# MPI-SWS/RedQueen

Hardware: AMD Instinct MI355X
Metric: redqueen_replicas_per_sec (higher is better)
Workload: dtype f64; 1 GPU; C3 syn1k: 1000 followers, 50 sources (25 Poisson2 rate 1 + 25 Hawkes l0=1 a=1 b=10), degree 5, T=100, q=1e6, s=1, RedQueen, randomized worlds; replicas_per_gpu=10000, global_batch=10000, parallelism=replica-sharded dp1, replicas_per_chunk=10000

## Files before the change

redqueen_amd/csrc/rq_api.cpp:

```cpp
#include <hip/hip_runtime.h>

#include <algorithm>
#include <cstring>
#include <memory>
#include <mutex>
#include <new>
#include <vector>

#include "../../include/rq.h"
#include "rq_internal.h"

using rqh::align_up;
using rqh::CtrlTables;
using rqh::GraphTopo;
using rqh::Knobs;
using rqh::Plan;

namespace {

template <class T>
struct DevBuf {
    T* p = nullptr;
    size_t n = 0;
    ~DevBuf() { if (p) (void)hipFree(p); }
// ... 562 lines not shown
    if (!g || !ids) return RQ_EINVAL;
    std::copy(g->fol_ids.begin(), g->fol_ids.end(), ids);
    return RQ_OK;
}

int rq_workspace_size(rq_graph_t g, const rq_batch_desc* b, size_t* bytes)
{
    if (!bytes) return RQ_EINVAL;
    Plan p;
    const int rc = plan_call(g, b, rqh::read_knobs(), 0.0, &p);
    if (rc) return rc;
    *bytes = p.total;
    return RQ_OK;
}

int rq_plan_info(rq_graph_t g, const rq_batch_desc* b, int64_t* info)
{
    return rq_plan_info_n(g, b, info, 8);
}

int rq_plan_info_n(rq_graph_t g, const rq_batch_desc* b, int64_t* out, int n)
{
    if (!out || n < 0) return RQ_EINVAL;
    int64_t info[10];
    Plan p;
    const int rc = plan_call(g, b, rqh::read_knobs(), 0.0, &p);
    if (rc) return rc;
    rqh::plan_info(p, b->ctrl_kind, info);
    info[9] = p.blk ? 1 : 0;
    std::copy(info, info + std::min(n, 10), out);
    return RQ_OK;
}

int rq_event_capacity(rq_graph_t g, const rq_batch_desc* b, int64_t* cap)
{
    if (!cap) return RQ_EINVAL;
    Plan p;
    const int rc = plan_call(g, b, rqh::read_knobs(), 0.0, &p);
    if (rc) return rc;
    *cap = p.cap_rows;
    return RQ_OK;
}

int rq_run_batch(rq_graph_t g, const rq_batch_desc* b, const rq_outputs* out, void* workspace,
                 size_t workspace_bytes, void* hip_stream)
{
    const Knobs kn = rqh::read_knobs();
    Plan p;
    int rc = plan_call(g, b, kn, (double)workspace_bytes, &p);
    if (rc) return rc;
    if (!out || !out->metrics || !out->counts || !out->status || !workspace) return RQ_EINVAL;
    if (workspace_bytes < p.total) return RQ_EINVAL;
    if ((b->flags & RQ_RUN_EVENT_LOG) && (!out->ev_t || !out->ev_src || out->ev_cap < 1))
// ... 4 lines not shown
    if ((rc = stage_tables(g, p, b, rqh::ctrl_tables(*g, b), ws, pst[0]))) return rc;
    if (hipMemsetAsync(out->status, 0, sizeof(int32_t) * p.R, pst[0]) != hipSuccess) return RQ_EHIP;
    Join join{pst, t_pipes.of(pst[0])};
    if ((rc = fork_streams(p.nbuf, &join))) return rc;

    int64_t ci = 0;
    for (int64_t c0 = 0; c0 < p.R; c0 += p.chunk, ++ci) {
        hipStream_t s = pst[ci % p.nbuf];
        const Chunk ch{c0, std::min(p.chunk, p.R - c0), ws,
                       ws + p.off_set0 + (size_t)(ci % p.nbuf) * p.set_stride};
        const GenArgs ga = gen_args(g, p, b, out, ch, kn);
        if (!p.fw || p.fwm) {
            TimedLaunch tl(K_GEN, s);
            if (rq_launch_gen(ga, s) != hipSuccess) return RQ_EHIP;
        }
        if (p.mrg && (rc = launch_merge(p, merge_args(g, p, out, ch, ga, kn), ch, s))) return rc;
        const SweepArgs sa = sweep_args(g, p, b, out, ch, ga, kn);
        if (p.order && rq_launch_order(sa.mrg_len, ch.C, (int*)(ch.wsb + p.off_ord), s) != hipSuccess)
            return RQ_EHIP;
        if (hipMemsetAsync(ch.wsb + p.off_wq, 0, 2 * sizeof(int), s) != hipSuccess) return RQ_EHIP;
        {
            TimedLaunch tl(K_SWEEP, s);
            const SweepInst inst = rqh::sweep_inst(p, b->ctrl_kind);
            const hipError_t e = inst.fused ? rq_launch_sweep_fw(sa, inst, s) : rq_launch_sweep(sa, inst, s);
            if (e != hipSuccess) return RQ_EHIP;
        }
        if (p.scan) continue;
        const ScanArgs sc = scan_args(g, p, out, ch, sa);
        TimedLaunch tl(K_SCAN, s);
        if (rq_launch_scan(sc, p.nK, s) != hipSuccess) return RQ_EHIP;
    }
    return join.done();
}

int rq_timing(int enable)
{
    for (int k = 0; k < K_N; ++k) {
        for (auto& e : g_ev[k]) {
            (void)hipEventDestroy(e.first);
            (void)hipEventDestroy(e.second);
        }
        g_ev[k].clear();
    }
    g_timing = enable != 0;
    return RQ_OK;
}

// ... 762 lines not shown
```

redqueen_amd/csrc/rq_host.h:

```cpp
#pragma once
#include <stddef.h>
#include <stdint.h>

#include <vector>

#include "../../include/rq.h"

#define RQ_MAX_STREAMS 2048
#define RQ_NPSUM1_LDS 516
#ifndef RQ_MRG_LB
#define RQ_MRG_LB 1024
#endif
#define RQ_MG_B 512
#define RQ_MAX_STREAMS_MRG (RQ_MG_B * RQ_MG_B)

struct SweepInst {
    bool fused;
    int nK;
    bool col16;
    bool log;
    bool gs;
    bool bits;
    bool bl;
    bool mrg;
    int spl;
    int W;
    bool gt;
    bool pw;
    bool pair;
    bool scan;
    bool blk;
};
#define RQ_BLK_CB(nw) ((((nw) + 7) >> 3) << 1)
#define RQ_BLK_MSTRIDE(nw) (4 * RQ_BLK_CB(nw) + 4)
#define RQ_BLK_MIN_NW 13
#define RQ_FWS_NL 66
#define RQ_FWS_LDS_BYTES(nK) ((size_t)8 * (((nK) + 2 + 3) * RQ_FWS_NL + 4))

#ifndef RQ_FOLLOWERS_TILE_SINKS
#define RQ_FOLLOWERS_TILE_SINKS 2048
#endif
static_assert(RQ_FOLLOWERS_TILE_SINKS >= 1 &&
                  (long long)RQ_FOLLOWERS_TILE_SINKS * (12 + 8 * (RQ_MAX_K + 2) + 8) <= 160 * 1024,
              "a tile of every nK / rows variant must fit one workgroup's LDS");

int rq_sweep_blocks_per_cu(const SweepInst& i, int wpb, size_t lds);
int rq_fw_blocks_per_cu(const SweepInst& i, int wpb, size_t lds);
int rq_cu_count();

namespace rqh {

inline size_t align_up(size_t x, size_t a) { return (x + a - 1) / a * a; }

inline int followers_tiles(int n_sinks) { return (n_sinks + RQ_FOLLOWERS_TILE_SINKS - 1) / RQ_FOLLOWERS_TILE_SINKS; }
inline size_t followers_tiled_ws_bytes(int n_sinks, int64_t n_rep)
{
    return align_up((size_t)4 * (size_t)n_rep * (size_t)followers_tiles(n_sinks), 256);
}

template <class T>
struct Knob {
    bool set = false;
    T v{};
};
struct Knobs {
    Knob<double> ws_budget_gb;
    double cap_squeeze = 1.0;
    Knob<int> mg_grp;
    bool mrg = true;
    Knob<int> g_collds;
    int g_w = 0;
    bool skip = true;
    bool fwm = true;
    bool ctrl_draws = true;
    bool sweep_scan = true;
    bool gen_split = true;
    bool phasec_blk = true;
    int fw_w = 0;
    int pipe = 2;
    Knob<int64_t> pipe_chunk;
    bool order = false;

    int sweep_dbg = 0;
    double fw_tile = 58.0;
    Knob<int> fw_hmin, fw_thr, fw_hfill;
    int fw_static = 0;
    bool clk_merge = false;

    Knob<int> rp_chunk;
    bool rp_small = true;
    bool clk_replay = false;

    int lm_of_slots = 4096;
};
Knobs read_knobs();

struct GraphTopo {
    int n_str = 0, ctrl_idx = -1, n_sinks = 0, n_fol = 0;
// ... 31 lines not shown
    std::vector<int> cap;
    std::vector<int64_t> st_off;
    std::vector<int> rd_k;
    bool log = false, bits = false;
    bool bl = false;
    size_t g_fb = 0, g_etab = 0, g_inv = 0, g_skip = 0;
    bool g_inv_sh = false;
    bool gs = false;
    int64_t gs_slots = 0, gs_stride = 0;
    bool fw = false;
    int fw_h = 8, mstride = 1;
    bool mrg = false;
    bool lmrg = false;
    bool gt = false;
    size_t off_mt = 0, off_mj = 0, off_mjh = 0, off_mlen = 0;
    int64_t mrg_stride = 0;
    int n_grp = 1;
    int grp_sz = RQ_MG_B;
    int64_t sub_stride = 0;
    size_t off_sub_t = 0, off_sub_j = 0, off_sub_len = 0;
    bool fwm = false;
    bool pair = false;
    bool scan = false;
    bool blk = false;
    int gwpb = 4, gwin = 16, gcol_lds = 1, gcol16 = 0;
    size_t g_col = 0, g_ptr = 0, g_odf = 0, g_cbf = 0, g_wave = 0, g_wave_stride = 0, g_rank_off = 0,
           g_win_off = 0, g_x_off = 0, g_total = 0, g_stage_off = 0;
    size_t tables_bytes = 0;
    int wpc = 0;
    int nbuf = 1;
    bool order = false;
    size_t off_set0 = 0, set_stride = 0, off_ord = 0;
    size_t off_pwc = 0, off_pwmax = 0;
    size_t off_invc = 0, off_streams = 0, off_slen = 0, off_rt = 0, off_rs = 0, off_rv = 0,
           off_rc = 0, off_sall = 0, off_wq = 0, off_stoff = 0, off_cap = 0, off_rdk = 0, off_repidx = 0, off_gs = 0,
           total = 0;
};

int make_plan(const GraphTopo& g, const rq_batch_desc* b, const Knobs& kn, double budget, Plan* p);
SweepInst sweep_inst(const Plan& p, int ctrl_kind);
void plan_info(const Plan& p, int ctrl_kind, int64_t info[9]);

struct CtrlTables {
    std::vector<double> invc;
    std::vector<double> pwc, pwmax;
};
// ... 35 lines not shown
```

redqueen_amd/csrc/rq_internal.h:

```cpp
#pragma once
#include <hip/hip_runtime.h>
#include <stdint.h>

#include <map>
#include <mutex>
#include <tuple>

#include "../../include/rq.h"
#include "rq_host.h"
#include "rq_log_walk.h"

__host__ __device__ __forceinline__ int64_t rq_global_replica(int64_t s, int64_t n_rep, int64_t rep_lo,
                                                               int64_t rep_cnt)
{
    return rep_cnt == n_rep ? s : (s / rep_cnt) * n_rep + rep_lo + s % rep_cnt;
}

struct GenArgs {
    int64_t n_chunk, chunk0, rep0;
    int64_t n_rep, rep_lo, rep_cnt;
    const int64_t* rep_idx;
    int n_str, ctrl_idx, ctrl_stream_kind, randomize;
    int64_t seed_mod;
    const uint32_t* ctrl_seed;
// ... 135 lines not shown
    int64_t n_chunk, chunk0;
    const int64_t* nrows;
    int64_t nrows_stride;
    const int* sall;
    int64_t row_stride;
    const double* rows_t;
    const double* rows_sum;
    const uint32_t* rows_valid;
    const uint32_t* rows_cnt;
    double end;
    double* metrics;
    int* wq;
};

using SweepKernel = void (*)(SweepArgs);

hipError_t rq_launch_gen(const GenArgs& a, hipStream_t s);
hipError_t rq_launch_sweep(const SweepArgs& a, const SweepInst& i, hipStream_t s);
hipError_t rq_launch_scan(const ScanArgs& a, int nK, hipStream_t s);
hipError_t rq_launch_merge(const MergeArgs& a, hipStream_t s);
hipError_t rq_launch_merge_groups(const MergeArgs& a, hipStream_t s);
hipError_t rq_launch_merge_sub(const MergeArgs& a, hipStream_t s);
hipError_t rq_launch_order(const int* len, int64_t n, int* order, hipStream_t s);
hipError_t rq_launch_sweep_fw(const SweepArgs& a, const SweepInst& i, hipStream_t s);

template <class K>
int rq_occupancy(K kernel, int threads, size_t lds)
{
    static std::mutex mu;
    static std::map<std::tuple<const void*, int, size_t>, int> cache;
    const auto key = std::make_tuple(reinterpret_cast<const void*>(kernel), threads, lds);
    std::lock_guard<std::mutex> lock(mu);
    const auto it = cache.find(key);
    if (it != cache.end()) return it->second;
    int nb = 0;
    if (hipOccupancyMaxActiveBlocksPerMultiprocessor(&nb, kernel, threads, lds) != hipSuccess) nb = 0;
    cache.emplace(key, nb);
    return nb;
}

struct RpInfo {
    int64_t n_piv;
    int64_t n_own, n_world;
    int32_t S;
    int32_t flags;
};
#define RP_FALLBACK 1
// ... 277 lines not shown
```

redqueen_amd/csrc/rq_plan.cpp:

```cpp
#include <algorithm>
#include <cmath>
#include <cstdlib>

#include "rq_host.h"
#include "rq_tables.h"

namespace rqh {

Knobs read_knobs()
{
    Knobs k;
    if (const char* e = getenv("RQ_WS_BUDGET_GB")) k.ws_budget_gb = {true, atof(e)};
    if (const char* e = getenv("RQ_CAP_SQUEEZE")) k.cap_squeeze = std::max(0.01, std::min(1.0, atof(e)));
    if (const char* e = getenv("RQ_MG_GRP")) k.mg_grp = {true, atoi(e)};
    if (const char* e = getenv("RQ_MRG")) k.mrg = atoi(e) != 0;
    if (const char* e = getenv("RQ_G_COLLDS")) k.g_collds = {true, atoi(e)};
    if (const char* e = getenv("RQ_G_W")) k.g_w = atoi(e);
    if (const char* e = getenv("RQ_SKIP")) k.skip = atoi(e) != 0;
    if (const char* e = getenv("RQ_FWM")) k.fwm = atoi(e) != 0;
    if (const char* e = getenv("RQ_CTRL_DRAWS")) k.ctrl_draws = atoi(e) != 0;
    if (const char* e = getenv("RQ_SWEEP_SCAN")) k.sweep_scan = atoi(e) != 0;
    if (const char* e = getenv("RQ_GEN_SPLIT")) k.gen_split = atoi(e) != 0;
    if (const char* e = getenv("RQ_PHASEC_BLK")) k.phasec_blk = atoi(e) != 0;
    if (const char* e = getenv("RQ_FW_W")) k.fw_w = atoi(e);
    if (const char* e = getenv("RQ_PIPE")) k.pipe = std::max(1, std::min(3, atoi(e)));
    if (const char* e = getenv("RQ_PIPE_CHUNK")) k.pipe_chunk = {true, std::max<int64_t>(64, atoll(e))};
    if (const char* e = getenv("RQ_ORDER")) k.order = atoi(e) != 0;
    if (const char* e = getenv("RQ_SWEEP_DBG")) k.sweep_dbg = atoi(e);
    if (const char* e = getenv("RQ_FW_TILE")) k.fw_tile = atof(e);
    if (const char* e = getenv("RQ_FW_HMIN")) k.fw_hmin = {true, atoi(e)};
    if (const char* e = getenv("RQ_FW_THR")) k.fw_thr = {true, atoi(e)};
    if (const char* e = getenv("RQ_FW_HFILL")) k.fw_hfill = {true, atoi(e)};
    static const int fw_static = getenv("RQ_FW_STATIC") ? atoi(getenv("RQ_FW_STATIC")) : 0;
    k.fw_static = fw_static;
    k.clk_merge = getenv("RQ_CLK_MERGE") != nullptr;
    if (const char* e = getenv("RQ_RP_CHUNK")) k.rp_chunk = {true, atoi(e)};
    if (const char* e = getenv("RQ_RP_SMALL")) k.rp_small = atoi(e) != 0;
    k.clk_replay = getenv("RQ_CLK_REPLAY") != nullptr;
    if (const char* e = getenv("RQ_LM_OF_SLOTS")) k.lm_of_slots = std::max(1, std::min(4096, atoi(e)));
    return k;
}

namespace {

// ... 42 lines not shown
        break;
    }
    return m;
}

SweepInst sweep_inst(const Plan& p, int ctrl_kind, bool fused, int W, bool col16, bool gs, bool gt)
{
    SweepInst i{};
    i.fused = fused;
    i.nK = p.nK;
    i.col16 = col16;
    i.log = p.log;
    i.gs = gs;
    i.bits = p.bits;
    i.bl = p.bl;
    i.mrg = fused ? p.fwm : p.mrg;
    i.spl = p.spl;
    i.W = W;
    i.gt = gt;
    i.pw = ctrl_kind == RQ_SRC_OPTPW;
    i.pair = fused && i.mrg && p.pair;
    i.scan = fused && i.mrg && p.scan;
    i.blk = fused && i.mrg && p.blk;
    return i;
}
int sweep_blocks_per_cu(const SweepInst& i, int wpb, size_t lds)
{
    return i.fused ? rq_fw_blocks_per_cu(i, wpb, lds) : rq_sweep_blocks_per_cu(i, wpb, lds);
}

void plan_layout(const GraphTopo* g, const rq_batch_desc* b, Plan* p);

int plan_args(const GraphTopo* g, const rq_batch_desc* b, Plan* p)
{
    if (!b) return RQ_EINVAL;
    if (b->nK < 1 || b->nK > RQ_MAX_K || !b->Ks) return RQ_EINVAL;
    if (b->n_grid < 1 || b->n_rep < 1) return RQ_EINVAL;
    const int ck = b->ctrl_kind;
    if (ck != RQ_SRC_OPT && ck != RQ_SRC_OPTPW && ck != RQ_SRC_POISSON2 && ck != RQ_SRC_PWCONST &&
        ck != RQ_SRC_REALDATA && ck != RQ_SRC_NONE)
        return RQ_EINVAL;
    if (ck == RQ_SRC_OPT && (!b->q || (g->n_fol > 0 && !b->s))) return RQ_EINVAL;
    if (ck == RQ_SRC_OPTPW &&
        (!b->q || b->n_seg < 1 || b->n_seg > 4096 || !(b->period > 0.0) || (g->n_fol > 0 && !b->s_pw)))
        return RQ_EINVAL;
    if (ck == RQ_SRC_POISSON2 && !b->ctrl_rate) return RQ_EINVAL;
// ... 218 lines not shown
            if (p->scan) stride = std::max(stride, align_up(RQ_FWS_LDS_BYTES(p->nK), 16));
            for (int wpb : {16, 12, 10, 8, 6, 5, 4, 3, 2, 1}) {
                const size_t tot = sh + wpb * stride;
                if (tot > kLdsMax) continue;
                int blocks = sweep_blocks_per_cu(sweep_inst(*p, b->ctrl_kind, true, W, c16, false, false), wpb, tot);
                if (blocks <= 0) blocks = (int)std::min<size_t>(kLdsMax / tot, 16 / wpb);
                const int waves = blocks * wpb;
                const int score = waves * 4 + (W == 16 ? 2 : W == 32 ? 1 : 0);
                if (score > best) {
                    best = score;
                    p->wpc = waves;
                    p->gwin = W; p->fw_h = H; p->gwpb = wpb; p->gcol_lds = c16; p->gcol16 = c16;
                    p->g_col = o_col; p->g_ptr = o_ptr; p->g_odf = o_odf; p->g_cbf = o_cbf;
                    p->g_wave = sh; p->g_wave_stride = stride; p->g_rank_off = r_off;
                    p->g_win_off = w_off; p->g_stage_off = s_off; p->g_x_off = 0; p->g_total = tot;
                    p->g_etab = o_etab;
                }
            }
        }
        if (best < 0) p->fw = false;
    }
    if (!p->fw) p->fwm = false;
    if (!p->fwm) p->pair = p->scan = p->blk = false;
    if (p->blk) p->mstride = mstride;
    if (p->fw) p->mrg = p->fwm;
}

}

SweepInst sweep_inst(const Plan& p, int ctrl_kind)
{
    return sweep_inst(p, ctrl_kind, p.fw, p.gwin, p.gcol16, p.gs, p.gt);
}

void plan_info(const Plan& p, int ctrl_kind, int64_t info[9])
{
    info[0] = (p.log ? (p.gs ? 4 : 1) : (p.bits ? 2 : (p.bl ? 3 : 0))) + (p.fwm ? 20 : p.fw ? 10 : 0);
    info[1] = p.mrg ? 0 : p.spl;
    info[2] = p.gwin;
    info[3] = p.gwpb;
    info[4] = sweep_blocks_per_cu(sweep_inst(p, ctrl_kind), p.gwpb, p.g_total);
    info[5] = p.gcol_lds;
    info[6] = (int64_t)p.g_total;
    info[7] = p.chunk;
    info[8] = p.scan ? 1 : 0;
}
// ... 133 lines not shown
```

redqueen_amd/csrc/rq_scan_rows.h:

```cpp
#pragma once
#include <hip/hip_runtime.h>
#include <stdint.h>

#include "rq_device.h"

#pragma clang fp contract(off)

namespace rq {

template <int NK, int TU, int NL = 128>
__device__ __forceinline__ void scan_rows(int64_t n, double S, double end, const double* Rt, const double* Rs,
                                          const uint32_t* Rv, const uint32_t* Rc, double* lds,
                                          double res[NK + 2])
{
    constexpr int NV = NK + 2;
    struct Row {
        double t, s;
        uint32_t v, c[NK];
    };
    auto ld = [&](uint32_t kk) {
        Row r;
        r.t = Rt[kk];
        r.s = Rs[kk];
        r.v = Rv[kk];
#pragma unroll
        for (int q = 0; q < NK; ++q) r.c[q] = Rc[kk * NK + q];
        return r;
    };
    auto tld = [&](uint32_t kk) { return Rt[kk]; };
    auto vf = [&](const Row& r, double t1, double* v) {
        const double dt = t1 - r.t;
        const double m = r.s / (double)r.v;
#pragma unroll
        for (int q = 0; q < NK; ++q) v[q] = ((double)r.c[q] / S) * dt;
        v[NK] = m * dt;
        v[NK + 1] = (m * m) * dt;
    };
    wave_npsum_rows<NV, true, Row, TU, NL>(n, end, ld, tld, vf, lds, res);
}

}
```

redqueen_amd/csrc/rq_sweep_core.h:

```cpp
#pragma once
#include "rq_device.h"
#include "rq_internal.h"

namespace rq {
static_assert(npsum_lds_doubles<1>() == RQ_NPSUM1_LDS, "wave_npsum<1> scratch size (rq_api.cpp plans it)");

template <int NK>
struct Agg {
    int64_t sumR, sumF;
    int nvalid;
    int cnt[NK];
    int km1[NK];
    __device__ __forceinline__ void init(const int* Ks)
    {
        sumR = 0;
        sumF = 0;
        nvalid = 0;
#pragma unroll
        for (int q = 0; q < NK; ++q) {
            cnt[q] = 0;
            km1[q] = Ks[q] - 1;
        }
    }
    template <class RT, class CF>
// ... 260 lines not shown
            nvalid += popc(__ballot(nv));
            nfrac += popc(__ballot(fup)) - popc(__ballot(fdn));
#pragma unroll
            for (int q = 0; q < NK; ++q) cnt[q] += popc(__ballot(up[q])) - popc(__ballot(dn[q]));
#pragma unroll
            for (int o = 32; o > 0; o >>= 1) dsum += __shfl_xor(dsum, o, 64);
            sumI += dsum;
        }
    }
    __device__ __forceinline__ double row_sum(int n_sinks, double* lds)
    {
        if (nfrac == 0) return (double)sumI;
        double out[1];
        wave_npsum<1>((int64_t)n_sinks,
                      [&](int64_t kk, double* v) {
                          const int c = (int)kk;
                          v[0] = gtag[c] >= 0 ? (double)gsum[c] / (double)gcnt[c] : 0.0;
                      },
                      lds, out);
        return out[0];
    }
};

template <int NK>
struct RowStage {
    double r_t, r_sum;
    int r_valid;
    int r_cnt[NK];
    int64_t nrow, s0, cap;
    double last_t;
    double* Rt0;
    double* Rs0;
    uint32_t* Rv0;
    uint32_t* Rc0;
    int64_t rb;
    uint32_t p_o, p_w;
    double p_ot, p_os, p_wt, p_ws;
    int p_ov, p_wv;
    int p_oc[NK], p_wc[NK];
    __device__ __forceinline__ void init(double* t, double* s, uint32_t* v, uint32_t* c, int64_t rb_,
                                         int64_t cap_)
    {
        p_o = p_w = ~0u;
        r_t = 0.0;
        r_sum = 0.0;
        r_valid = 0;
#pragma unroll
// ... 34 lines not shown
#pragma unroll
            for (int q = 0; q < NK; ++q) r_cnt[q] = cnt[q];
        }
        ++nrow;
        last_t = t;
        if (slot == 63) {
            store(s0 + lane);
            s0 = nrow;
        }
        return true;
    }
    __device__ __forceinline__ void store(int64_t rr) { write(rr, r_t, r_sum, r_valid, r_cnt); }
    __device__ __forceinline__ void flush_pend()
    {
        if (p_o != ~0u) write(p_o, p_ot, p_os, p_ov, p_oc);
        if (p_w != ~0u) write(p_w, p_wt, p_ws, p_wv, p_wc);
        p_o = p_w = ~0u;
    }
    __device__ __forceinline__ void flush(int lane)
    {
        const int rem = (int)(nrow - s0);
        if (lane < rem) store(s0 + lane);
        s0 = nrow;
    }
};

__device__ __forceinline__ double optpw_sample(double tt, const double* row, double smax, int S,
                                               double T, uint64_t e, uint32_t oseed)
{
    if (!(smax > 0.0)) return RQ_INF;
    const double inv = 1.0 / smax;
    const double ph = fmod(tt, T);
    double ns = 0.0;
    for (uint32_t it = 1; it < (1u << 20); ++it) {
        uint32_t w4[4] = {(uint32_t)e, (uint32_t)(e >> 32), it, 0u};
        philox4x32_10(w4, oseed, kind_salt(RQ_SRC_OPTPW, true));
        ns = ns + rq_std_exponential(rq_uniform53(w4[0], w4[1])) * inv;
        int idx = (int)(((double)S * fmod(ns + ph, T)) / T);
        idx = idx < S ? idx : S - 1;
        if (rq_uniform53(w4[2], w4[3]) * smax < row[idx]) return tt + ns;
    }
    return RQ_INF;
}

template <bool PW, bool XIN = false>
__device__ __forceinline__ void controller_tile(int n, bool act, double tt, int tj, const double* invc,
// ... 44 lines not shown
}

__device__ __forceinline__ bool truncate_tile(int64_t M, int64_t n_events, int& n, bool& act, double& tt,
                                              int& tj, uint64_t& ownm, double ot, double& opt_next)
{
    if (M < 0) return false;
    const int lane = lane_id();
    const int64_t pp = n_events + lane + mbcnt64(ownm);
    const int64_t pw = pp + (int64_t)((ownm >> lane) & 1ull);
    const int nk = __popcll(__ballot(act && pw < M));
    if (nk >= n) return false;
    const bool lone = ((ownm >> nk) & 1ull) != 0ull && bcast_i64(pp, nk) < M;
    opt_next = lone ? bcast_d(ot, nk) : RQ_INF;
    ownm &= nk > 0 ? (~0ull >> (64 - nk)) : 0ull;
    n = nk;
    act = lane < nk;
    if (!act) {
        tt = RQ_INF;
        tj = 0;
    }
    return true;
}

template <int NK, bool DEFER = false>
__device__ __forceinline__ bool place_rows(RowStage<NK>& rs, uint64_t ma, bool has_o, bool has_w, double ot,
                                           double tt, int64_t osum, int oval, const int* ocnt,
                                           int64_t wsum, int wval, const int* wcnt, int& status)
{
    const int lane = lane_id();
    const uint64_t mo = __ballot(has_o), mw = __ballot(has_w);
    const uint64_t above = lane < 63 ? ma >> (lane + 1) : 0ull;
    const bool nxt = above != 0;
    const double ft = has_o ? ot : tt;
    const double nft = __shfl(ft, nxt ? lane + __ffsll((unsigned long long)above) : lane, 64);
    const bool keep_o = has_o && !(has_w ? ot == tt : (nxt && ot == nft));
    const bool keep_w = has_w && !(nxt && tt == nft);
    const bool tie0 = rs.nrow > 0 && bcast_d(ft, __ffsll((unsigned long long)ma) - 1) == rs.last_t;
    const uint64_t ko = __ballot(keep_o), kw = __ballot(keep_w);
    if (tie0 || ko != mo || kw != mw) status |= RQ_ST_TIE;
    const int64_t r0 = rs.nrow - (tie0 ? 1 : 0);
    const int64_t po = r0 + mbcnt64(ko) + mbcnt64(kw);
    const int64_t pw = po + (keep_o ? 1 : 0);
    if constexpr (DEFER) {
        rs.p_o = keep_o && po < rs.cap ? (uint32_t)po : ~0u;
        rs.p_w = keep_w && pw < rs.cap ? (uint32_t)pw : ~0u;
        rs.p_ot = ot;
        rs.p_os = (double)osum;
        rs.p_ov = oval;
        rs.p_wt = tt;
        rs.p_ws = (double)wsum;
        rs.p_wv = wval;
#pragma unroll
        for (int q = 0; q < NK; ++q) {
            rs.p_oc[q] = ocnt[q];
            rs.p_wc[q] = wcnt[q];
        }
    } else {
        if (keep_o && po < rs.cap) rs.write(po, ot, (double)osum, oval, ocnt);
        if (keep_w && pw < rs.cap) rs.write(pw, tt, (double)wsum, wval, wcnt);
    }
    rs.last_t = bcast_d(has_w ? tt : ot, 63 - __builtin_clzll(ma));
    rs.nrow = r0 + __popcll(ko) + __popcll(kw);
    rs.s0 = rs.nrow;
    if (rs.nrow > rs.cap) {
        rs.nrow = rs.cap;
        rs.s0 = rs.cap;
// ... 52 lines not shown
```

redqueen_amd/csrc/rq_sweep_fw.hip:

```cpp
#include <hip/hip_runtime.h>
#include <stdint.h>

#include "rq_device.h"
#include "rq_internal.h"
#include "rq_sweep_core.h"
#include "rq_gen.h"
#include "rq_scan_rows.h"
#include <type_traits>
#include <cstdlib>

#pragma clang fp contract(off)

using namespace rq;

constexpr int fws_tu(int nk) { return nk == 1 ? 4 : 2; }
template <int NK>
__device__ __forceinline__ void fw_scan_rows(int64_t n, double S, double end, const double* Rt, const double* Rs,
                                             const uint32_t* Rv, const uint32_t* Rc, double* lds, double* out)
{
    constexpr int NV = NK + 2;
    static_assert(RQ_FWS_LDS_BYTES(NK) == 8 * (size_t)npsum_lds_doubles<NV, RQ_FWS_NL>(), "the planner's size");
    const int lane = lane_id();
    if (n == 0) {
        if (lane < NV) out[lane] = __builtin_nan("");
        return;
    }
    __asm__ volatile("s_waitcnt vmcnt(0)" ::: "memory");
    __builtin_amdgcn_fence(__ATOMIC_RELEASE, "workgroup");
    __builtin_amdgcn_fence(__ATOMIC_ACQUIRE, "workgroup");
    double res[NV];
    scan_rows<NK, fws_tu(NK), RQ_FWS_NL>(n, S, end, Rt, Rs, Rv, Rc, lds, res);
    if (lane == 0) {
#pragma unroll
        for (int s = 0; s < NV; ++s) out[s] = res[s];
    }
}
template <int NK, class COL, int W, int H, bool BITS, bool PW, bool MRG, bool PAIR = false, bool SCAN = false,
          bool BLK = false>
__device__ __forceinline__ void sweep_fw_body(SweepArgs a)
{
    static_assert((W & (W - 1)) == 0 && H <= W, "ring");
    static_assert(!SCAN || MRG, "the sweep's own scan: merged instances only");
    static_assert(!BLK || (MRG && BITS), "event-blocked phase C: the merged sink-bit instances only");
    extern __shared__ double lds_g[];
    char* base = reinterpret_cast<char*>(lds_g);
    const int lane = lane_id();
    const int w = threadIdx.x >> 6;
    int* cptr = reinterpret_cast<int*>(base + a.lds_ptr);
    int* odf = reinterpret_cast<int*>(base + a.lds_odf);
    int* cbf = reinterpret_cast<int*>(base + a.lds_cbf);
    constexpr bool col_lds = sizeof(COL) == 2;
    COL* col_l = reinterpret_cast<COL*>(base + a.lds_col);
    const int* col_g = a.csr_col;
    if (col_lds && !BITS)
        for (int e = threadIdx.x; e < a.n_csr; e += blockDim.x) col_l[e] = (COL)a.csr_col[e];
    uint32_t* msk = reinterpret_cast<uint32_t*>(base + a.lds_mask);
    const int ms = a.mstride;
    if (BITS)
        for (int e = threadIdx.x; e < (a.n_str + 1) * ms; e += blockDim.x) {
            const int jj = e / ms, ww = e - jj * ms;
            msk[e] = (jj < a.n_str && ww < a.nw) ? a.masks[jj * a.nw + ww] : 0u;
        }
    uint64_t* etab = reinterpret_cast<uint64_t*>(base + a.lds_etab);
    for (int e = threadIdx.x; e < RQ_EXP_TAB_N; e += blockDim.x) etab[e] = rq_exp_tab_c[e];
    for (int j = threadIdx.x; j <= a.n_str; j += blockDim.x) cptr[j] = a.csr_ptr[j];
    for (int j = threadIdx.x; j < a.n_str; j += blockDim.x) {
// ... 13 lines not shown
    const int64_t rl = a.order ? (int64_t)a.order[qi] : qi;
    const int64_t o = a.chunk0 + rl;
    const int64_t i = rq_replica_of(a.gen, o);
    const int g = (int)(i / a.n_rep);
    for (int j = lane; j < a.n_str; j += 64) invc[j] = a.inv_c[(int64_t)g * a.n_str + j];
    if (!BITS)
        for (int c = lane; c < a.n_sinks; c += 64) rank[c] = -1;
    wave_lds_sync();

#ifdef RQ_PHASE_CLOCK
    unsigned long long ck[8] = {0, 0, 0, 0, 0, 0, 0, 0};
    unsigned long long tk = __builtin_amdgcn_s_memtime();
#define RQ_CLK(q)                                                   \
    do {                                                            \
        const unsigned long long t2 = __builtin_amdgcn_s_memtime(); \
        ck[q] += t2 - tk;                                           \
        tk = t2;                                                    \
    } while (0)
#else
#define RQ_CLK(q) \
    do {          \
    } while (0)
#endif
    constexpr bool DEFER = MRG && RQ_MRG_DEFER;
    SrcGen gen;
    if (lane < a.n_str && !MRG) gen.init(a.gen, lane, i, etab);
    else gen.none();
    int pos = 0, fil = 0;
    const int64_t mb = MRG ? rl * a.mrg_stride : 0;
    auto mload = [&](int64_t e, double& t_, int& j_) __attribute__((always_inline)) {
        int64_t x = mb;
        __asm__ volatile("" : "+v"(x));
        t_ = a.mrg_t[x + e];
        j_ = a.mrg_j[x + e];
    };
    const int mlen = MRG ? a.mrg_len[rl] : 0;
    int mpos = 0;
    double nxt_t = RQ_INF;
    int nxt_j = 0;
    if (MRG && lane < mlen) mload(lane, nxt_t, nxt_j);

    const bool opt = a.ctrl_kind == RQ_SRC_OPT || a.ctrl_kind == RQ_SRC_OPTPW;
    const double* pwc = PW ? a.pw_c + (size_t)g * a.n_str * a.n_seg : nullptr;
    const double* pwm = PW ? a.pw_max + (size_t)g * a.n_str : nullptr;
    double opt_next = opt ? a.start : RQ_INF;
    const int64_t k = a.seed_mod > 0 ? i % a.seed_mod : i;
    const uint32_t oseed = a.ctrl_seed ? a.ctrl_seed[i] : a.ctrl_seed0 + (uint32_t)k;
    uint64_t ndraw = 0;
    double px0 = 0.0, px1 = 0.0;
    auto colat = [&](int e) -> int { return col_lds ? (int)col_l[e] : col_g[e]; };
    const int fol0 = cptr[a.ctrl_idx];
    auto folat = [&](int f) -> int { return colat(fol0 + f); };

    Agg<NK> ag;
    ag.init(a.Ks);
    AggB agb;
    if (BITS) {
        agb.init(msk, a.nw, ms, a.ctrl_idx, lane);
        if (lane < (BLK ? 4 * RQ_BLK_CB(a.nw) : (a.nw + 1) & ~1)) ft[lane] = make_uint2(agb.F, 0u);
    }
    RowStage<NK> rs;
    const int64_t rbase = rl * a.cap_rows;
    rs.init(a.rows_t, a.rows_sum, a.rows_valid, a.rows_cnt, rbase, a.cap_rows);

    int64_t n_events = 0, posts = 0, world = 0;
    int status = 0;
    double span = -1.0;
    bool stop = false;
    const int thr = a.fw_thr;
    auto refill_pass = [&]() __attribute__((always_inline)) {
#ifdef RQ_PHASE_CLOCK
        ck[6] += 1;
        ck[7] += __popcll(__ballot(!gen.done && fil - pos < W));
#endif
        if (!gen.done && fil - pos < W) {
            double tv;
            if (gen.step(&tv, a.end)) {
                ring[fil & (W - 1)] = tv;
                ++fil;
            }
        }
    };
    for (;;) {
        int n = 0;
// ... 275 lines not shown
                        oval = ag.nvalid;
#pragma unroll
                        for (int kq = 0; kq < NK; ++kq) ocnt[kq] = ag.cnt[kq];
                    }
                }
                const int jw = bcast_i(tj, q);
                if (!opt && jw == a.ctrl_idx)
                    ag.own(rank, folat, a.n_fol, lane);
                else
                    ag.wall(rank, colat, bcast_i(e0, q), bcast_i(e1, q), bcast_i(od, q), lane);
                if (lane == q) {
                    wsum = ag.sumR;
                    wval = ag.nvalid;
#pragma unroll
                    for (int kq = 0; kq < NK; ++kq) wcnt[kq] = ag.cnt[kq];
                }
            }
        }
        RQ_CLK(4);
        const uint64_t mo = __ballot(has_o), ma = mo | __ballot(has_w);
        n_events += n + __popcll(ownm);
        posts += __popcll(mo) + __popcll(__ballot(has_w && strm_own));
        world += __popcll(__ballot(has_w && !strm_own));
        if (ma && place_rows<NK, DEFER>(rs, ma, has_o, has_w, ot, tt, osum, oval, ocnt, wsum, wval, wcnt, status))
            stop = true;
        RQ_CLK(5);
        if (stop || fin) break;
    }
    if constexpr (DEFER) rs.flush_pend();
#ifdef RQ_PHASE_CLOCK
    if (lane == 0 && a.clk)
        for (int q = 0; q < 8; ++q) atomicAdd(&a.clk[q], ck[q]);
#endif
    if (BITS) agb.T = lane < a.nw ? ft[lane].y : 0u;
    if (!stop && opt && opt_next <= a.end && (a.max_events < 0 || n_events < a.max_events)) {
        if (a.ev_t && lane == 0) {
            if (n_events < a.ev_cap) {
                a.ev_t[o * a.ev_cap + n_events] = opt_next;
                a.ev_src[o * a.ev_cap + n_events] = a.ctrl_idx;
            } else {
                status |= RQ_ST_ROWS_OVERFLOW;
            }
        }
        ++n_events;
        if (BITS) {
            agb.own();
            agb.sync();
// ... 17 lines not shown
                rs.s0 = rs.nrow;
                rs.last_t = opt_next;
            }
            if (rr >= 0 && lane == 0) {
                rs.write(rr, opt_next, (double)ag.sumR, ag.nvalid, ag.cnt);
            }
        }
    }
    if (BITS) {
        agb.sync();
        ag.nvalid = agb.nvalid;
    }
    if (lane == 0) {
        int64_t* cnto = a.counts + o * 4;
        cnto[0] = posts;
        cnto[1] = world;
        cnto[2] = n_events;
        cnto[3] = rs.nrow;
        a.sall[rl] = ag.nvalid;
        if (rs.nrow == 0) status |= RQ_ST_EMPTY;
        if (status) atomicOr(&a.status[o], status);
    }
    if constexpr (SCAN)
        fw_scan_rows<NK>(rs.nrow, (double)ag.nvalid, a.end, a.rows_t + rbase, a.rows_sum + rbase,
                         a.rows_valid + rbase, a.rows_cnt + rbase * NK, reinterpret_cast<double*>(wb),
                         a.metrics + o * (NK + 2));
    if (!a.wq) break;
    int nx = 0;
    if (lane == 0) nx = atomicAdd(a.wq, 1);
    qi = nslot + __builtin_amdgcn_readfirstlane(nx);
    }
}

template <int NK, class COL, int W, int H, bool BITS, bool PW = false, bool MRG = false>
__global__ __launch_bounds__(1024) void rq_sweep_fw(SweepArgs a)
{
    sweep_fw_body<NK, COL, W, H, BITS, PW, MRG>(a);
}
#ifndef RQ_FWM_WPE
#define RQ_FWM_WPE 4
#endif
template <int NK, class COL, bool BITS, bool PAIR = false, bool SCAN = false, bool BLK = false>
__global__ __launch_bounds__(1024) __attribute__((amdgpu_waves_per_eu(RQ_FWM_WPE))) void rq_sweep_fwm(SweepArgs a)
{
    sweep_fw_body<NK, COL, 16, 8, BITS, false, true, PAIR, SCAN, BLK>(a);
}

template <class COL, int W, bool PW = false>
static SweepKernel fw_nk(int nK)
{
    constexpr int H = W > 16 ? 8 : W / 2;
    switch (nK) {
    case 1: return rq_sweep_fw<1, COL, W, H, false, PW>;
    case 2: return rq_sweep_fw<2, COL, W, H, false, PW>;
    case 3: return rq_sweep_fw<3, COL, W, H, false, PW>;
    default: return rq_sweep_fw<4, COL, W, H, false, PW>;
    }
}
template <class COL, bool PAIR, bool SCAN>
static SweepKernel fwm_nk(int nK)
{
    switch (nK) {
    case 1: return rq_sweep_fwm<1, COL, false, PAIR, SCAN>;
    case 2: return rq_sweep_fwm<2, COL, false, PAIR, SCAN>;
    case 3: return rq_sweep_fwm<3, COL, false, PAIR, SCAN>;
    default: return rq_sweep_fwm<4, COL, false, PAIR, SCAN>;
    }
}
template <bool PAIR, bool SCAN>
static SweepKernel fwm_kernel(const SweepInst& i)
{
    if (i.blk && !i.bits) return nullptr;
    if (i.bits)
        return i.blk ? rq_sweep_fwm<1, uint16_t, true, PAIR, SCAN, true> : rq_sweep_fwm<1, uint16_t, true, PAIR, SCAN>;
    return i.col16 ? fwm_nk<uint16_t, PAIR, SCAN>(i.nK) : fwm_nk<int, PAIR, SCAN>(i.nK);
}
static SweepKernel fw_kernel(const SweepInst& i)
{
    if (i.mrg) {
        if (i.pw) return nullptr;
        if (i.pair)
            return i.scan ? fwm_kernel<true, true>(i) : fwm_kernel<true, false>(i);
        return i.scan ? fwm_kernel<false, true>(i) : fwm_kernel<false, false>(i);
    }
    if (i.pair || i.scan || i.blk) return nullptr;
    if (i.pw) {
        if (!i.col16 || i.W != 16) return nullptr;
        return i.bits ? rq_sweep_fw<1, uint16_t, 16, 8, true, true> : fw_nk<uint16_t, 16, true>(i.nK);
    }
    if (i.bits)
        return i.W == 32 ? rq_sweep_fw<1, uint16_t, 32, 8, true>
             : i.W == 16 ? rq_sweep_fw<1, uint16_t, 16, 8, true> : rq_sweep_fw<1, uint16_t, 8, 4, true>;
    if (i.W == 16) return i.col16 ? fw_nk<uint16_t, 16>(i.nK) : fw_nk<int, 16>(i.nK);
    return i.col16 ? fw_nk<uint16_t, 8>(i.nK) : fw_nk<int, 8>(i.nK);
}

static int occ_fw_t(SweepKernel k, int wpb, size_t lds)
{
    return rq_occupancy(k, 64 * wpb, lds);
}
static hipError_t launch_fw_t(SweepKernel k, const SweepArgs& a, hipStream_t s)
{
    unsigned blocks = (unsigned)((a.n_chunk + a.wpb - 1) / a.wpb);
    if (a.wq) {
        const int nb = occ_fw_t(k, a.wpb, a.lds_total);
        const unsigned cap = (unsigned)(nb > 0 ? nb : 1) * (unsigned)rq_cu_count();
        if (cap < blocks) blocks = cap;
    }
    hipLaunchKernelGGL(k, dim3(blocks), dim3(64 * a.wpb), a.lds_total, s, a);
    return hipGetLastError();
}

hipError_t rq_launch_sweep_fw(const SweepArgs& a, const SweepInst& i, hipStream_t s)
{
    if (a.n_chunk <= 0) return hipSuccess;
    if (i.pair && a.ctrl_kind != RQ_SRC_OPT) return hipErrorInvalidValue;
    if (i.scan && (!a.metrics || a.ev_t || a.max_events >= 0 || a.lds_wave_stride < RQ_FWS_LDS_BYTES(i.nK)))
        return hipErrorInvalidValue;
    if (i.blk && a.mstride != RQ_BLK_MSTRIDE(a.nw)) return hipErrorInvalidValue;
    const SweepKernel k = fw_kernel(i);
    return k ? launch_fw_t(k, a, s) : hipErrorInvalidValue;
}

int rq_fw_blocks_per_cu(const SweepInst& i, int wpb, size_t lds)
{
    const SweepKernel k = fw_kernel(i);
    return k ? occ_fw_t(k, wpb, lds) : -1;
}
```

redqueen_amd/engine.py:

```python
import ctypes as C
import math

import numpy as np
import torch

from . import _lib as L

KIND_BY_NAME = {"Poisson": L.SRC_POISSON, "Poisson2": L.SRC_POISSON2, "Hawkes": L.SRC_HAWKES,
                "PiecewiseConst": L.SRC_PWCONST, "RealData": L.SRC_REALDATA, "Opt": L.SRC_OPT}
CTRL_BY_NAME = {"opt": L.SRC_OPT, "poisson": L.SRC_POISSON2, "pwconst": L.SRC_PWCONST,
                "times": L.SRC_REALDATA, "wall": L.SRC_NONE, "sig": L.SRC_OPTPW}


def _arr(x, dt):
    return np.ascontiguousarray(np.asarray(x, dtype=dt))


def _source_class(name):
    if isinstance(name, str):
        if name in KIND_BY_NAME:
            return None
        from .opt_model import SimOpts
        cls = SimOpts.broadcasters.get(name)
        if cls is None:
# ... 246 lines not shown
            b.ctrl_rate = cr.data_ptr()
            b.ctrl_rate_max = float(cr.max().item()) if cr.numel() else 0.0
        b.Ks = Ks.ctypes.data_as(L._pi32)
        b.nK = Ks.size
        b.max_events = -1 if max_events is None or max_events == float("inf") else int(max_events)
        b.flags = L.RUN_EVENT_LOG if event_log else 0
        b.cap_scale = float(cap_scale)
        b.chunk = int(chunk)
        b.sweep_mode = int(sweep_mode)
        b.replica0 = int(replica0)
        b.n_local = int(n_local)
        b.rep_lo = lo
        b.rep_cnt = int(rep_cnt)
        if rep_idx is not None:
            keep.append(gids)
            b.rep_idx = gids.ctypes.data_as(L._pi64)
        if spw is not None:
            b.n_seg = spw.shape[2]
            b.period = float(period)
            b.s_pw = spw.ctypes.data_as(L._pd)
        lib = L.lib()
        if plan_only:
            b.ws_budget = self._ws_budget(dev)
            info = (C.c_int64 * 10)()
            L.check("rq_plan_info_n", lib.rq_plan_info_n(self._h, C.byref(b), info, 10))
            keys = ("variant", "sources_per_lane", "ring_depth", "waves_per_block",
                    "blocks_per_cu", "columns_in_lds", "lds_bytes_per_block", "chunk", "sweep_scan",
                    "sweep_blk")
            return dict(zip(keys, (int(v) for v in info)))
        return self._run_loop(lib, b, keep, dev, R, Ks, n_grid, n_rep, ck, event_log,
                              gids, check, stream)

    @property
    def player_ids(self):
        return [p["src_id"] for p in self.players]

    def _player_s(self, src_id, s):
        fol = sorted({int(e[1]) for e in self._edges if int(e[0]) == int(src_id)})
        if isinstance(s, dict):
            return np.asarray([s[x] for x in fol], dtype=np.float64)
        return np.ascontiguousarray(np.ones(len(fol), dtype=np.float64) * np.asarray(s, dtype=np.float64))

    GAME_REPLAY_ROWS = 1 << 26
    GAME_CAP_SQUEEZE = 1.0
    GAME_METRICS = "log"
    GAME_METRICS_SLIM = True
    game_metrics_route = None

    def _game_launch(self, players, seeds, ev_t, ev_src, counts, max_events, out_cap, use):
        lib = L.lib()
        dev = ev_t.device
# ... 921 lines not shown
```

Baseline: 4.976 million replicas/s.

## Pack sweep scan rows into 16-byte records for single-K merged sweeps

When the fused merged sweep does its own scan with one K, each event row is written as one 16-byte uint4 (time, 32-bit sum, 16-bit valid and count) instead of being spread over separate time, sum, valid and count arrays. The scan then reads each row with a single vector load and uses a larger unroll. This cuts the number of memory transactions on the row write/read path, but the row stage can no longer defer writes, and the layout only applies when the sink count and merge stride fit in 16/32 bits.

```diff
diff --git a/redqueen_amd/csrc/rq_api.cpp b/redqueen_amd/csrc/rq_api.cpp
--- a/redqueen_amd/csrc/rq_api.cpp
+++ b/redqueen_amd/csrc/rq_api.cpp
@@ -608,13 +608,14 @@
 int rq_plan_info_n(rq_graph_t g, const rq_batch_desc* b, int64_t* out, int n)
 {
     if (!out || n < 0) return RQ_EINVAL;
-    int64_t info[10];
+    int64_t info[11];
     Plan p;
     const int rc = plan_call(g, b, rqh::read_knobs(), 0.0, &p);
     if (rc) return rc;
     rqh::plan_info(p, b->ctrl_kind, info);
     info[9] = p.blk ? 1 : 0;
-    std::copy(info, info + std::min(n, 10), out);
+    info[10] = p.rows16 ? 1 : 0;
+    std::copy(info, info + std::min(n, 11), out);
     return RQ_OK;
 }
 
@@ -665,7 +666,8 @@
         {
             TimedLaunch tl(K_SWEEP, s);
             const SweepInst inst = rqh::sweep_inst(p, b->ctrl_kind);
-            const hipError_t e = inst.fused ? rq_launch_sweep_fw(sa, inst, s) : rq_launch_sweep(sa, inst, s);
+            const hipError_t e = inst.fused ? rq_launch_sweep_fw(sa, inst, s, p.off_rv - p.off_rt)
+                                            : rq_launch_sweep(sa, inst, s);
             if (e != hipSuccess) return RQ_EHIP;
         }
         if (p.scan) continue;
diff --git a/redqueen_amd/csrc/rq_host.h b/redqueen_amd/csrc/rq_host.h
--- a/redqueen_amd/csrc/rq_host.h
+++ b/redqueen_amd/csrc/rq_host.h
@@ -30,6 +30,7 @@
     bool pair;
     bool scan;
     bool blk;
+    bool pk;
 };
 #define RQ_BLK_CB(nw) ((((nw) + 7) >> 3) << 1)
 #define RQ_BLK_MSTRIDE(nw) (4 * RQ_BLK_CB(nw) + 4)
@@ -51,6 +52,12 @@
 namespace rqh {
 
 inline size_t align_up(size_t x, size_t a) { return (x + a - 1) / a * a; }
+
+inline bool rows16_fits(int nK, int n_sinks, int64_t mrg_stride)
+{
+    return nK == 1 && n_sinks >= 0 && n_sinks <= 65535 && mrg_stride >= 0 && mrg_stride < ((int64_t)1 << 32) &&
+           (uint64_t)n_sinks * (uint64_t)mrg_stride < ((uint64_t)1 << 32);
+}
 
 inline int followers_tiles(int n_sinks) { return (n_sinks + RQ_FOLLOWERS_TILE_SINKS - 1) / RQ_FOLLOWERS_TILE_SINKS; }
 inline size_t followers_tiled_ws_bytes(int n_sinks, int64_t n_rep)
@@ -74,6 +81,7 @@
     bool fwm = true;
     bool ctrl_draws = true;
     bool sweep_scan = true;
+    bool rows_packed = true;
     bool gen_split = true;
     bool phasec_blk = true;
     int fw_w = 0;
@@ -151,6 +159,7 @@
     bool fwm = false;
     bool pair = false;
     bool scan = false;
+    bool rows16 = false;
     bool blk = false;
     int gwpb = 4, gwin = 16, gcol_lds = 1, gcol16 = 0;
     size_t g_col = 0, g_ptr = 0, g_odf = 0, g_cbf = 0, g_wave = 0, g_wave_stride = 0, g_rank_off = 0,
diff --git a/redqueen_amd/csrc/rq_internal.h b/redqueen_amd/csrc/rq_internal.h
--- a/redqueen_amd/csrc/rq_internal.h
+++ b/redqueen_amd/csrc/rq_internal.h
@@ -181,7 +181,7 @@
 hipError_t rq_launch_merge_groups(const MergeArgs& a, hipStream_t s);
 hipError_t rq_launch_merge_sub(const MergeArgs& a, hipStream_t s);
 hipError_t rq_launch_order(const int* len, int64_t n, int* order, hipStream_t s);
-hipError_t rq_launch_sweep_fw(const SweepArgs& a, const SweepInst& i, hipStream_t s);
+hipError_t rq_launch_sweep_fw(const SweepArgs& a, const SweepInst& i, hipStream_t s, size_t rows16_bytes = 0);
 
 template <class K>
 int rq_occupancy(K kernel, int threads, size_t lds)
diff --git a/redqueen_amd/csrc/rq_plan.cpp b/redqueen_amd/csrc/rq_plan.cpp
--- a/redqueen_amd/csrc/rq_plan.cpp
+++ b/redqueen_amd/csrc/rq_plan.cpp
@@ -20,6 +20,7 @@
     if (const char* e = getenv("RQ_FWM")) k.fwm = atoi(e) != 0;
     if (const char* e = getenv("RQ_CTRL_DRAWS")) k.ctrl_draws = atoi(e) != 0;
     if (const char* e = getenv("RQ_SWEEP_SCAN")) k.sweep_scan = atoi(e) != 0;
+    if (const char* e = getenv("RQ_ROWS_PACKED")) k.rows_packed = atoi(e) != 0;
     if (const char* e = getenv("RQ_GEN_SPLIT")) k.gen_split = atoi(e) != 0;
     if (const char* e = getenv("RQ_PHASEC_BLK")) k.phasec_blk = atoi(e) != 0;
     if (const char* e = getenv("RQ_FW_W")) k.fw_w = atoi(e);
@@ -108,6 +109,7 @@
     i.pair = fused && i.mrg && p.pair;
     i.scan = fused && i.mrg && p.scan;
     i.blk = fused && i.mrg && p.blk;
+    i.pk = i.scan && p.rows16;
     return i;
 }
 int sweep_blocks_per_cu(const SweepInst& i, int wpb, size_t lds)
@@ -372,6 +374,8 @@
     }
     if (!p->fw) p->fwm = false;
     if (!p->fwm) p->pair = p->scan = p->blk = false;
+    p->rows16 = p->scan && rows16_fits(p->nK, g->n_sinks, p->mrg_stride);
+    p->rows16 = p->rows16 && kn.rows_packed;
     if (p->blk) p->mstride = mstride;
     if (p->fw) p->mrg = p->fwm;
 }
diff --git a/redqueen_amd/csrc/rq_scan_rows.h b/redqueen_amd/csrc/rq_scan_rows.h
--- a/redqueen_amd/csrc/rq_scan_rows.h
+++ b/redqueen_amd/csrc/rq_scan_rows.h
@@ -8,16 +8,44 @@
 
 namespace rq {
 
+template <int NK>
+struct ScanRow {
+    double t, s;
+    uint32_t v, c[NK];
+    __device__ __forceinline__ double sum() const { return s; }
+    __device__ __forceinline__ uint32_t valid() const { return v; }
+    __device__ __forceinline__ uint32_t cnt(int q) const { return c[q]; }
+};
+struct ScanRow16 {
+    double t;
+    uint32_t su, cv;
+    __device__ __forceinline__ double sum() const { return (double)su; }
+    __device__ __forceinline__ uint32_t valid() const { return cv >> 16; }
+    __device__ __forceinline__ uint32_t cnt(int) const { return cv & 0xFFFFu; }
+};
+
+template <int NK, int TU, int NL, class Row, class LD, class TLD>
+__device__ __forceinline__ void scan_rows_of(int64_t n, double S, double end, LD&& ld, TLD&& tld, double* lds,
+                                             double res[NK + 2])
+{
+    constexpr int NV = NK + 2;
+    auto vf = [&](const Row& r, double t1, double* v) {
+        const double dt = t1 - r.t;
+        const double m = r.sum() / (double)r.valid();
+#pragma unroll
+        for (int q = 0; q < NK; ++q) v[q] = ((double)r.cnt(q) / S) * dt;
+        v[NK] = m * dt;
+        v[NK + 1] = (m * m) * dt;
+    };
+    wave_npsum_rows<NV, true, Row, TU, NL>(n, end, ld, tld, vf, lds, res);
+}
+
 template <int NK, int TU, int NL = 128>
 __device__ __forceinline__ void scan_rows(int64_t n, double S, double end, const double* Rt, const double* Rs,
                                           const uint32_t* Rv, const uint32_t* Rc, double* lds,
                                           double res[NK + 2])
 {
-    constexpr int NV = NK + 2;
-    struct Row {
-        double t, s;
-        uint32_t v, c[NK];
-    };
+    using Row = ScanRow<NK>;
     auto ld = [&](uint32_t kk) {
         Row r;
         r.t = Rt[kk];
@@ -28,15 +56,23 @@
         return r;
     };
     auto tld = [&](uint32_t kk) { return Rt[kk]; };
-    auto vf = [&](const Row& r, double t1, double* v) {
-        const double dt = t1 - r.t;
-        const double m = r.s / (double)r.v;
-#pragma unroll
-        for (int q = 0; q < NK; ++q) v[q] = ((double)r.c[q] / S) * dt;
-        v[NK] = m * dt;
-        v[NK + 1] = (m * m) * dt;
+    scan_rows_of<NK, TU, NL, Row>(n, S, end, ld, tld, lds, res);
+}
+
+template <int TU, int NL = 128>
+__device__ __forceinline__ void scan_rows16(int64_t n, double S, double end, const uint4* R, double* lds,
+                                            double res[3])
+{
+    auto ld = [&](uint32_t kk) {
+        const uint4 x = R[kk];
+        ScanRow16 r;
+        r.t = rq_bits_dbl(((uint64_t)x.y << 32) | x.x);
+        r.su = x.z;
+        r.cv = x.w;
+        return r;
     };
-    wave_npsum_rows<NV, true, Row, TU, NL>(n, end, ld, tld, vf, lds, res);
+    auto tld = [&](uint32_t kk) { return reinterpret_cast<const double*>(R + kk)[0]; };
+    scan_rows_of<1, TU, NL, ScanRow16>(n, S, end, ld, tld, lds, res);
 }
 
 }
diff --git a/redqueen_amd/csrc/rq_sweep_core.h b/redqueen_amd/csrc/rq_sweep_core.h
--- a/redqueen_amd/csrc/rq_sweep_core.h
+++ b/redqueen_amd/csrc/rq_sweep_core.h
@@ -306,7 +306,7 @@
     }
 };
 
-template <int NK>
+template <int NK, bool PK = false>
 struct RowStage {
     double r_t, r_sum;
     int r_valid;
@@ -387,6 +387,36 @@
         const int rem = (int)(nrow - s0);
         if (lane < rem) store(s0 + lane);
         s0 = nrow;
+    }
+};
+
+__device__ __forceinline__ uint32_t row16_cv(int valid, int cnt) { return (uint32_t)cnt | ((uint32_t)valid << 16); }
+template <int NK>
+struct RowStage<NK, true> {
+    static_assert(NK == 1, "16-byte rows: one K");
+    int64_t nrow, s0, cap;
+    double last_t;
+    uint4* R0;
+    int64_t rb;
+    __device__ __forceinline__ void init(double* t, double*, uint32_t*, uint32_t*, int64_t rb_, int64_t cap_)
+    {
+        nrow = 0;
+        s0 = 0;
+        cap = cap_;
+        last_t = -RQ_INF;
+        R0 = reinterpret_cast<uint4*>(t);
+        rb = rb_;
+    }
+    __device__ __forceinline__ void write16(int64_t rr, double t, uint32_t sum, uint32_t cv)
+    {
+        int64_t b = rb;
+        __asm__ volatile("" : "+v"(b));
+        const uint64_t tb = rq_dbl_bits(t);
+        R0[b + rr] = make_uint4((uint32_t)tb, (uint32_t)(tb >> 32), sum, cv);
+    }
+    __device__ __forceinline__ void write(int64_t rr, double t, double sum, int valid, const int* cnt)
+    {
+        write16(rr, t, (uint32_t)sum, row16_cv(valid, cnt[0]));
     }
 };
 
@@ -477,8 +507,8 @@
     return true;
 }
 
-template <int NK, bool DEFER = false>
-__device__ __forceinline__ bool place_rows(RowStage<NK>& rs, uint64_t ma, bool has_o, bool has_w, double ot,
+template <int NK, bool DEFER = false, bool PK = false>
+__device__ __forceinline__ bool place_rows(RowStage<NK, PK>& rs, uint64_t ma, bool has_o, bool has_w, double ot,
                                            double tt, int64_t osum, int oval, const int* ocnt,
                                            int64_t wsum, int wval, const int* wcnt, int& status)
 {
@@ -496,7 +526,11 @@
     const int64_t r0 = rs.nrow - (tie0 ? 1 : 0);
     const int64_t po = r0 + mbcnt64(ko) + mbcnt64(kw);
     const int64_t pw = po + (keep_o ? 1 : 0);
-    if constexpr (DEFER) {
+    if constexpr (PK) {
+        static_assert(!DEFER, "16-byte rows are not deferred");
+        if (keep_o && po < rs.cap) rs.write16(po, ot, (uint32_t)osum, row16_cv(oval, ocnt[0]));
+        if (keep_w && pw < rs.cap) rs.write16(pw, tt, (uint32_t)wsum, row16_cv(wval, wcnt[0]));
+    } else if constexpr (DEFER) {
         rs.p_o = keep_o && po < rs.cap ? (uint32_t)po : ~0u;
         rs.p_w = keep_w && pw < rs.cap ? (uint32_t)pw : ~0u;
         rs.p_ot = ot;
diff --git a/redqueen_amd/csrc/rq_sweep_fw.hip b/redqueen_amd/csrc/rq_sweep_fw.hip
--- a/redqueen_amd/csrc/rq_sweep_fw.hip
+++ b/redqueen_amd/csrc/rq_sweep_fw.hip
@@ -13,8 +13,8 @@
 
 using namespace rq;
 
-constexpr int fws_tu(int nk) { return nk == 1 ? 4 : 2; }
-template <int NK>
+constexpr int fws_tu(int nk, bool pk = false) { return nk == 1 ? (pk ? 6 : 4) : 2; }
+template <int NK, bool PK = false>
 __device__ __forceinline__ void fw_scan_rows(int64_t n, double S, double end, const double* Rt, const double* Rs,
                                              const uint32_t* Rv, const uint32_t* Rc, double* lds, double* out)
 {
@@ -29,19 +29,23 @@
     __builtin_amdgcn_fence(__ATOMIC_RELEASE, "workgroup");
     __builtin_amdgcn_fence(__ATOMIC_ACQUIRE, "workgroup");
     double res[NV];
-    scan_rows<NK, fws_tu(NK), RQ_FWS_NL>(n, S, end, Rt, Rs, Rv, Rc, lds, res);
+    if constexpr (PK)
+        scan_rows16<fws_tu(NK, true), RQ_FWS_NL>(n, S, end, reinterpret_cast<const uint4*>(Rt), lds, res);
+    else
+        scan_rows<NK, fws_tu(NK), RQ_FWS_NL>(n, S, end, Rt, Rs, Rv, Rc, lds, res);
     if (lane == 0) {
 #pragma unroll
         for (int s = 0; s < NV; ++s) out[s] = res[s];
     }
 }
 template <int NK, class COL, int W, int H, bool BITS, bool PW, bool MRG, bool PAIR = false, bool SCAN = false,
-          bool BLK = false>
+          bool BLK = false, bool PK = false>
 __device__ __forceinline__ void sweep_fw_body(SweepArgs a)
 {
     static_assert((W & (W - 1)) == 0 && H <= W, "ring");
     static_assert(!SCAN || MRG, "the sweep's own scan: merged instances only");
     static_assert(!BLK || (MRG && BITS), "event-blocked phase C: the merged sink-bit instances only");
+    static_assert(!PK || (SCAN && NK == 1), "16-byte rows: the sweep's own rows at one K");
     extern __shared__ double lds_g[];
     char* base = reinterpret_cast<char*>(lds_g);
     const int lane = lane_id();
@@ -101,7 +105,7 @@
     do {          \
     } while (0)
 #endif
-    constexpr bool DEFER = MRG && RQ_MRG_DEFER;
+    constexpr bool DEFER = MRG && RQ_MRG_DEFER && !PK;
     SrcGen gen;
     if (lane < a.n_str && !MRG) gen.init(a.gen, lane, i, etab);
     else gen.none();
@@ -138,7 +142,7 @@
         agb.init(msk, a.nw, ms, a.ctrl_idx, lane);
         if (lane < (BLK ? 4 * RQ_BLK_CB(a.nw) : (a.nw + 1) & ~1)) ft[lane] = make_uint2(agb.F, 0u);
     }
-    RowStage<NK> rs;
+    RowStage<NK, PK> rs;
     const int64_t rbase = rl * a.cap_rows;
     rs.init(a.rows_t, a.rows_sum, a.rows_valid, a.rows_cnt, rbase, a.cap_rows);
 
@@ -460,7 +464,7 @@
         n_events += n + __popcll(ownm);
         posts += __popcll(mo) + __popcll(__ballot(has_w && strm_own));
         world += __popcll(__ballot(has_w && !strm_own));
-        if (ma && place_rows<NK, DEFER>(rs, ma, has_o, has_w, ot, tt, osum, oval, ocnt, wsum, wval, wcnt, status))
+        if (ma && place_rows<NK, DEFER, PK>(rs, ma, has_o, has_w, ot, tt, osum, oval, ocnt, wsum, wval, wcnt, status))
             stop = true;
         RQ_CLK(5);
         if (stop || fin) break;
@@ -524,9 +528,9 @@
         if (status) atomicOr(&a.status[o], status);
     }
     if constexpr (SCAN)
-        fw_scan_rows<NK>(rs.nrow, (double)ag.nvalid, a.end, a.rows_t + rbase, a.rows_sum + rbase,
-                         a.rows_valid + rbase, a.rows_cnt + rbase * NK, reinterpret_cast<double*>(wb),
-                         a.metrics + o * (NK + 2));
+        fw_scan_rows<NK, PK>(rs.nrow, (double)ag.nvalid, a.end, a.rows_t + (PK ? 2 : 1) * rbase, a.rows_sum + rbase,
+                             a.rows_valid + rbase, a.rows_cnt + rbase * NK, reinterpret_cast<double*>(wb),
+                             a.metrics + o * (NK + 2));
     if (!a.wq) break;
     int nx = 0;
     if (lane == 0) nx = atomicAdd(a.wq, 1);
@@ -542,10 +546,10 @@
 #ifndef RQ_FWM_WPE
 #define RQ_FWM_WPE 4
 #endif
-template <int NK, class COL, bool BITS, bool PAIR = false, bool SCAN = false, bool BLK = false>
+template <int NK, class COL, bool BITS, bool PAIR = false, bool SCAN = false, bool BLK = false, bool PK = false>
 __global__ __launch_bounds__(1024) __attribute__((amdgpu_waves_per_eu(RQ_FWM_WPE))) void rq_sweep_fwm(SweepArgs a)
 {
-    sweep_fw_body<NK, COL, 16, 8, BITS, false, true, PAIR, SCAN, BLK>(a);
+    sweep_fw_body<NK, COL, 16, 8, BITS, false, true, PAIR, SCAN, BLK, PK>(a);
 }
 
 template <class COL, int W, bool PW = false>
@@ -573,6 +577,17 @@
 static SweepKernel fwm_kernel(const SweepInst& i)
 {
     if (i.blk && !i.bits) return nullptr;
+    if (i.pk) {
+        if constexpr (SCAN) {
+            if (i.nK != 1) return nullptr;
+            if (i.bits)
+                return i.blk ? rq_sweep_fwm<1, uint16_t, true, PAIR, true, true, true>
+                             : rq_sweep_fwm<1, uint16_t, true, PAIR, true, false, true>;
+            return i.col16 ? rq_sweep_fwm<1, uint16_t, false, PAIR, true, false, true> : nullptr;
+        } else {
+            return nullptr;
+        }
+    }
     if (i.bits)
         return i.blk ? rq_sweep_fwm<1, uint16_t, true, PAIR, SCAN, true> : rq_sweep_fwm<1, uint16_t, true, PAIR, SCAN>;
     return i.col16 ? fwm_nk<uint16_t, PAIR, SCAN>(i.nK) : fwm_nk<int, PAIR, SCAN>(i.nK);
@@ -585,7 +600,7 @@
             return i.scan ? fwm_kernel<true, true>(i) : fwm_kernel<true, false>(i);
         return i.scan ? fwm_kernel<false, true>(i) : fwm_kernel<false, false>(i);
     }
-    if (i.pair || i.scan || i.blk) return nullptr;
+    if (i.pair || i.scan || i.blk || i.pk) return nullptr;
     if (i.pw) {
         if (!i.col16 || i.W != 16) return nullptr;
         return i.bits ? rq_sweep_fw<1, uint16_t, 16, 8, true, true> : fw_nk<uint16_t, 16, true>(i.nK);
@@ -613,13 +628,17 @@
     return hipGetLastError();
 }
 
-hipError_t rq_launch_sweep_fw(const SweepArgs& a, const SweepInst& i, hipStream_t s)
+hipError_t rq_launch_sweep_fw(const SweepArgs& a, const SweepInst& i, hipStream_t s, size_t rows16_bytes)
 {
     if (a.n_chunk <= 0) return hipSuccess;
     if (i.pair && a.ctrl_kind != RQ_SRC_OPT) return hipErrorInvalidValue;
     if (i.scan && (!a.metrics || a.ev_t || a.max_events >= 0 || a.lds_wave_stride < RQ_FWS_LDS_BYTES(i.nK)))
         return hipErrorInvalidValue;
     if (i.blk && a.mstride != RQ_BLK_MSTRIDE(a.nw)) return hipErrorInvalidValue;
+    if (i.pk && (!a.rows_t || ((uintptr_t)a.rows_t & 15) != 0 ||
+                 (uint64_t)rows16_bytes < (uint64_t)16 * (uint64_t)a.n_chunk * (uint64_t)a.cap_rows ||
+                 !rqh::rows16_fits(i.nK, a.n_sinks, a.mrg_stride)))
+        return hipErrorInvalidValue;
     const SweepKernel k = fw_kernel(i);
     return k ? launch_fw_t(k, a, s) : hipErrorInvalidValue;
 }
diff --git a/redqueen_amd/engine.py b/redqueen_amd/engine.py
--- a/redqueen_amd/engine.py
+++ b/redqueen_amd/engine.py
@@ -292,11 +292,11 @@
         lib = L.lib()
         if plan_only:
             b.ws_budget = self._ws_budget(dev)
-            info = (C.c_int64 * 10)()
-            L.check("rq_plan_info_n", lib.rq_plan_info_n(self._h, C.byref(b), info, 10))
+            info = (C.c_int64 * 11)()
+            L.check("rq_plan_info_n", lib.rq_plan_info_n(self._h, C.byref(b), info, 11))
             keys = ("variant", "sources_per_lane", "ring_depth", "waves_per_block",
                     "blocks_per_cu", "columns_in_lds", "lds_bytes_per_block", "chunk", "sweep_scan",
-                    "sweep_blk")
+                    "sweep_blk", "sweep_rows16")
             return dict(zip(keys, (int(v) for v in info)))
         return self._run_loop(lib, b, keep, dev, R, Ks, n_grid, n_rep, ck, event_log,
                               gids, check, stream)
```

Result: faster. 5.389 million replicas/s, median of 6 (+8.3%).
